# BosonHBC/BHRayTracer

Measured on AMD Instinct MI355X. Metric: Mrays/s (closest-hit + any-hit rays per second), with wall-clock per frame, higher is better.
Workload: dtype f32

## Files before the change

bhraytracer_amd/csrc/device_state.h:

```cpp
#pragma once
#include "dev_buf.h"

namespace bhrt {

struct DeviceQueues {
    hipStream_t stream = nullptr;
    hipEvent_t ev[2] = {nullptr, nullptr};
    hipStream_t stream2 = nullptr;
    std::vector<hipEvent_t> slow_events;
    hipStream_t stream3 = nullptr;
    hipEvent_t ev_shade = nullptr, ev_shadow[2] = {nullptr, nullptr};
    std::vector<hipEvent_t> ev_pool;
    DeviceQueues() = default;
    DeviceQueues(const DeviceQueues &) = delete;
    DeviceQueues &operator=(const DeviceQueues &) = delete;
    ~DeviceQueues()
    {
        if (ev_shade) (void)hipEventDestroy(ev_shade);
        for (int k = 0; k < 2; k++) if (ev_shadow[k]) (void)hipEventDestroy(ev_shadow[k]);
        if (stream3) (void)hipStreamDestroy(stream3);
        for (int k = 0; k < 2; k++) if (ev[k]) (void)hipEventDestroy(ev[k]);
        for (hipEvent_t e : ev_pool) (void)hipEventDestroy(e);
        for (hipEvent_t e : slow_events) (void)hipEventDestroy(e);
        if (stream2) (void)hipStreamDestroy(stream2);
// ... 22 lines not shown
            if (GatherSortPairs(nullptr, nullptr, nullptr, nullptr, cnt, nullptr, &sort_temp_bytes, 28, stream) != 0) { SetError("gather sort: temp size"); return BHRT_ERR_HIP; }
            BHRT_TRY(d_sort_temp.Reserve(std::max<size_t>(sort_temp_bytes, 16)));
            cap = cnt;
        }
        BHRT_TRY(d_cnt.Reserve(1));
        BHRT_TRY(d_cells.Reserve((size_t)BHRT_GATHER_CELLS + 1));
        BHRT_TRY(d_tile_sums.Reserve((size_t)(BHRT_GATHER_CELLS / kScanTile + kScanBlock)));
        return h_cnt ? BHRT_OK : h_cnt.Alloc(1);
    }
};

struct PhotonSlot {
    DevBuf<DPhoton> d_photons;
    uint32_t n_photons = 0;
    std::vector<HostPhoton> h_photons;
    DevBuf<float4> d_ph_hot, d_ph_cold, d_ph_dbox;
    PhotonMapDev pm = {};
    void Clear() { d_photons.Free(); d_ph_hot.Free(); d_ph_cold.Free(); d_ph_dbox.Free(); n_photons = 0; h_photons.clear(); pm = PhotonMapDev{}; }
};

struct DeviceState : DeviceQueues {
    int device = -1;
    uint32_t n_cus = 256;
    DevBuf<uint8_t> d_blob;
    DevBuf<int32_t> d_chain;
    DevBuf<float> d_aux;
    DevBuf<bhrt_texcolor> d_emission;
    bool emission_on = false;
    bool emission_textured = false;
    bool le_on = false;
    DevBuf<float> d_le;
    DevBuf<bhrt_material> d_mtl_ext;
    DevBuf<float> d_r0_ext;
    DevBuf<int32_t> d_fm_tab;
    FaceMtlTable fm = {nullptr, 0};
    DevScene S;
    ShutterInfo shutter = {};
    uint32_t cap_samples = 0, cap_rays = 0, cap_frames = 0;
    DevBuf<float> d_rayf[2];
    DevBuf<uint32_t> d_rayu[2];
    DevBuf<float> d_hitf;
    DevBuf<int32_t> d_hiti;
    DevBuf<float> d_shf;
    DevBuf<uint32_t> d_shu;
    DevBuf<uint32_t> d_fu;
    DevBuf<uint64_t> d_fcode;
    DevBuf<float> d_ff;
    DevBuf<float> d_samples;
    DevBuf<uint32_t> d_root;
    DevBuf<uint32_t> d_order;
    uint32_t order_shard_cap = 0;
    DevBuf<uint32_t> d_seg;
    DevBuf<uint32_t> d_park;
    DevBuf<float> d_slowf;
    DevBuf<uint32_t> d_slowu;
    DevBuf<float> d_shf2;
    DevBuf<uint32_t> d_shu2;
    DevBuf<uint32_t> d_order_sh;
    DevBuf<uint32_t> d_seg_sh;
    DevBuf<Counters> d_cnt_sh;
    DevBuf<Counters> d_cnt;
    PinnedBuf<HostCounters> h_pub;
    HostCounters *d_pub = nullptr;
    uint32_t pub_seq = 0;
    int timers = 0;
    struct PendingTimer { int e0, e1; double *acc; };
    std::vector<PendingTimer> ev_pending;
    std::vector<int> ev_free;
    PhotonSlot cmap, gmap;
    DevBuf<float> d_ph_frames;
    GatherWorkspace gw;
    struct Knobs {
        int stream_waves = -1;
        bool fused_camera = true;
        bool no_slow_queue = false;
        bool debug_slow = false, debug_gather = false, debug_drain = false;
        bool balance_host = false;
        int frame_cap = 0;
        int gather_lane_budget = 0;
        bool gather_counting_sort = false;
        bool shadow_overlap = true;
        bool fused_resolve = true;
        bool finish_misses = true;
        int gather_stats = 0;
        void FromEnv()
        {
            if (const char *e = getenv("BHRT_STREAM_WAVES")) stream_waves = atoi(e);
            if (const char *e = getenv("BHRT_FUSED_CAMERA")) fused_camera = atoi(e) != 0;
            no_slow_queue = getenv("BHRT_NO_SLOW_QUEUE") != nullptr;
            debug_slow = getenv("BHRT_DEBUG_SLOW") != nullptr; debug_gather = getenv("BHRT_DEBUG_GATHER") != nullptr; debug_drain = getenv("BHRT_DEBUG_DRAIN") != nullptr;
            if (const char *e = getenv("BHRT_PHOTON_BALANCE_HOST")) balance_host = atoi(e) != 0;
            if (const char *e = getenv("BHRT_GATHER_COUNTING_SORT")) gather_counting_sort = atoi(e) != 0;
            if (const char *e = getenv("BHRT_SHADOW_OVERLAP")) shadow_overlap = atoi(e) != 0;
            if (const char *e = getenv("BHRT_FUSED_RESOLVE")) fused_resolve = atoi(e) != 0;
            if (const char *e = getenv("BHRT_FINISH_MISSES")) finish_misses = atoi(e) != 0;
        }
    } knobs;
    uint64_t pass_hint_key = 0;
    uint32_t pass_hint = 0;
    uint64_t frames_seen_key = 0;
    double frames_seen = 0;
    size_t frame_px = 0;
    DevBuf<uint8_t> d_frame_rgb;
    DevBuf<float> d_frame_rad, d_frame_var;
    DevBuf<uint32_t> d_frame_cnt;
    DevBuf<uint8_t> d_ad;
    DevBuf<uint8_t> d_prog;
    uint64_t prog_session = 0;
    DevBuf<uint8_t> d_dn;
    DevBuf<float4> d_guides;
    struct MovingNodeSlot {
        PinnedBuf<uint32_t> h;
        DevBuf<uint32_t> d;
        hipEvent_t done = nullptr;
        bool used = false;
        MovingNodeSlot() = default;
        MovingNodeSlot(const MovingNodeSlot &) = delete;
        MovingNodeSlot &operator=(const MovingNodeSlot &) = delete;
        ~MovingNodeSlot() { if (done) (void)hipEventDestroy(done); }
    } moving_nodes[2];
    uint32_t moving_turn = 0;
    DevBuf<int32_t> d_moving_id;
    size_t api_cap = 0;
    DevBuf<float> d_api_f;
    DevBuf<int32_t> d_api_i;
};

void DestroyDeviceState(DeviceState *d)
{
    if (!d) return;
    if (d->device >= 0) (void)hipSetDevice(d->device);
    delete d;
}

}
```

bhraytracer_amd/csrc/kernels.hip:

```cpp
#include <hip/hip_runtime.h>

#include <stdlib.h>
#include <string.h>

#include <algorithm>
#include <type_traits>
#include <chrono>
#include <string>
#include <vector>

#include "bhrt.h"
#include "denoise.h"
#include "temporal.h"
#include "device_color24.h"
#include "device_photon.h"
#include "photon_host.h"
#include "scene_internal.h"

namespace bhrt {

#define HIP_CHECK(expr)                                                                                        \
    do {                                                                                                       \
        hipError_t e_ = (expr);                                                                                \
        if (e_ != hipSuccess) {                                                                                \
// ... 212 lines not shown
        else atomicOr(&cnt->overflow.v, 8u);
    }
}
__device__ inline uint32_t shading_class(uint32_t meta, const Hit &hit)
{
    const uint32_t kind = meta & 15u;
    const bool is_hit = hit.node >= 0;
    bool heavy = false;
    if (is_hit) {
        if (kind == RK_CAMERA) heavy = true;
        else if (kind == RK_GI) heavy = fabsf(hit.t) > BHRT_BIAS;
        else if (kind == RK_REFR_IN) heavy = hit.front != 0;
        else heavy = true;
    }
    return heavy ? RC_HEAVY : ((kind == RK_REFR_IN && is_hit) ? RC_MEDIUM : RC_LIGHT);
}
template <bool kTex>
__device__ inline void gi_miss(const DevScene &S, const float *gi_mult, float *gi, uint32_t owner, V3 d)
{
    const V3 mult = ld3i(gi_mult, owner);
    V3 outc = v3(0, 0, 0);
    if (d.x == d.y && d.x == 0) {
        outc = outc + v3(1.0f, 0.0f, 1.0f);
    } else {
        V3 env = (kTex ? sample_environment(S, S.environment, d) : ld3(S.environment.color)) * mult;
        if (!(isnan_f(env.x) || isnan_f(env.y) || isnan_f(env.z))) outc = outc + env;
    }
    if (isnan_f(outc.x)) outc = v3(1.0f, 0.0f, 1.0f);
    else outc = clamp_white(outc);
    st3(gi, owner, outc);
}

struct SlowQueue {
    RayQueue q;
    uint32_t cap;
};
constexpr uint32_t kSlowCap = 1u << 16;
template <bool kPark, bool kCamera, bool kMeshes = true>
__global__ void __launch_bounds__(kBlock) __attribute__((amdgpu_waves_per_eu(kPark ? 7 : 1, 8))) k_trace_closest(DevScene S, PassInfo P, RayQueue q, uint32_t n, int uniform_side, HitBuf h, RayOrder ord, Counters *cnt,
                                                          SlowQueue slow , const float *fin_gi_mult, float *fin_gi, uint32_t *fin_root)
{
    constexpr bool kFinish = kPark || !kMeshes;
    __shared__ bhrt_bvh_node nodelet[(kPark || !kMeshes) ? 1 : BHRT_LDS_NODES];
    const uint32_t i = blockIdx.x * blockDim.x + threadIdx.x;
    bool active = i < n;
    V3 o = v3(0, 0, 0), d = v3(0, 0, 1);
    uint32_t meta = 0;
    if (active) fetch_ray<kCamera>(S, P, q, i, o, d, meta);
    const bool has_meta = kCamera || q.meta;
    const int side = has_meta ? (int)((meta >> 4) & 3u) : uniform_side;
    const bool dead = has_meta && (meta & 15u) == RK_DEAD;
    Hit hit;
    uint32_t key = 0;
    bool is_slow = false;
    int parked = trace_closest<kMeshes>(S, o, d, side, hit, active && !dead, (kPark || !kMeshes) ? nullptr : nodelet, 0, kPark, kPark ? &key : nullptr,
                                        (uint16_t *)nullptr, 0, BHRT_LDS_NODES, kCamera, kPark ? &is_slow : nullptr);
    if (kPark && parked >= 0 && is_slow && slow.cap) {
        const uint32_t k = atomicAdd(&cnt->n_slow.v, 1u);
        if (k < slow.cap) {
            slow.q.ox[k] = o.x; slow.q.oy[k] = o.y; slow.q.oz[k] = o.z; slow.q.dx[k] = d.x; slow.q.dy[k] = d.y; slow.q.dz[k] = d.z;
            slow.q.frame[k] = kCamera ? i : q.frame[i];
            slow.q.meta[k] = meta;
            slow.q.rng_ctr[k] = (kCamera || (meta & 15u) == RK_GI) ? 0u : q.rng_ctr[i];
            active = false;
            parked = -1;
        }
    }
    if (kFinish && active && !dead && parked < 0 && hit.node < 0) {
        const uint32_t kind = meta & 15u;
        if (!kCamera && kind == RK_GI && fin_gi) {
            gi_miss<false>(S, fin_gi_mult, fin_gi, q.frame[i], d);
            active = false;
        } else if (kind == RK_CAMERA && fin_root) {
            uint32_t slot = i;
            if (!kCamera) slot = q.frame[i];
            fin_root[slot] = kNoRootFrame;
            active = false;
        }
    }
    if (active) { h.t[i] = hit.t; h.node[i] = hit.node; h.prim[i] = hit.prim; h.front[i] = hit.front | ((parked + 1) << 8); }
    if (kPark && parked >= 0) {
        ord.park_key[i] = key;
        if (!kCamera) ord.park_rank[i] = atomicAdd(&ord.park_bucket[key], 1u);
    }
    if (!ord.idx) return;
    uint32_t cls = RC_NONE;
    if (active && !dead) cls = parked >= 0 ? (uint32_t)RC_MESH : shading_class(meta, hit);
    file_ray(cls, i, (i >> 10) & (BHRT_ORDER_SHARDS - 1) , ord, cnt);
}
__device__ inline bool parked_entry(const RayOrder &ord, uint32_t b, uint32_t *s_seg, uint32_t &i, uint32_t first_entry = 0 )
{
    __syncthreads();
    if (threadIdx.x < 64) {
        const uint32_t l = threadIdx.x;
        const uint32_t a = l <= BHRT_ORDER_SHARDS ? ord.mesh_start[l] : 0xffffffffu;
        const uint32_t n_le = (uint32_t)__popcll(__ballot(l < BHRT_ORDER_SHARDS && a <= b));
        if (l == 0) *s_seg = n_le - 1;
    }
    __syncthreads();
    if (b >= ord.mesh_start[BHRT_ORDER_SHARDS]) return false;
    const uint32_t seg = *s_seg;
    const uint32_t local = (b - ord.mesh_start[seg]) * kBlock + first_entry + threadIdx.x;
    const bool active = local < ord.mesh_count[seg];
    i = active ? ord.idx[((size_t)RC_MESH * BHRT_ORDER_SHARDS + seg) * ord.shard_cap + local] : 0xffffffffu;
    return true;
}
#ifndef BHRT_XCD_LOCAL
#define BHRT_XCD_LOCAL 0
#endif
__device__ inline bool xcd_slice(uint32_t b, uint32_t nb, uint32_t &slice)
{
    slice = b;
#if BHRT_XCD_LOCAL
    constexpr uint32_t G = BHRT_XCD_LOCAL, span = 8 * G;
    const uint32_t chunk = b / span, in = b % span;
    if ((chunk + 1) * span <= nb) slice = chunk * span + (in & 7u) * G + (in >> 3);
#endif
    return b < nb;
}
__global__ void __launch_bounds__(kBlock) k_park_scatter(RayOrder ord)
{
    __shared__ uint32_t s_seg;
    uint32_t i;
    for (uint32_t b = blockIdx.x; parked_entry(ord, b, &s_seg, i); b += gridDim.x)
        if (i != 0xffffffffu) ord.park_sorted[ord.park_bucket[ord.park_key[i]] + ord.park_rank[i]] = i;
}
constexpr uint32_t kMeshNodelet = 256;
#ifndef BHRT_MESH_BLOCK
#define BHRT_MESH_BLOCK 64
#endif
constexpr int kMeshBlock = BHRT_MESH_BLOCK;
template <bool kCamera, int kPath, bool kLS = false>
__global__ void __launch_bounds__(kCamera ? kBlock : kMeshBlock, kPath == 1 ? 6 : 4 ) k_trace_mesh(DevScene S, PassInfo P, RayQueue q, HitBuf h, RayOrder ord, Counters *cnt)
{
    typedef typename std::conditional<kPath == 2, uint32_t, uint16_t>::type PathT;
    constexpr int kTB = kCamera ? kBlock : kMeshBlock;
    __shared__ bhrt_bvh_node nodelet[kPath ? 1 : kMeshNodelet];
    __shared__ PathT path[kPath ? 33 * kTB : 1];
    __shared__ uint32_t s_seg;
    bool active;
    uint32_t i;
    uint32_t slice;
    if (kCamera) {
        if (!xcd_slice(blockIdx.x, ord.mesh_start[BHRT_ORDER_SHARDS], slice)) return;
        if (!parked_entry(ord, slice, &s_seg, i)) return;
        active = i != 0xffffffffu;
        if (!active) i = 0;
    } else {
        const uint32_t total = ord.mesh_count[BHRT_ORDER_SHARDS];
        if (!xcd_slice(blockIdx.x, (total + kTB - 1) / kTB, slice)) return;
        const uint32_t k = slice * kTB + threadIdx.x;
        active = k < total;
        i = active ? ord.park_sorted[k] : 0u;
    }
    V3 o = v3(0, 0, 0), d = v3(0, 0, 1);
    uint32_t meta = 0;
    Hit hit = {BHRT_BIGFLOAT, -1, -1, 1};
    int start = 0;
    if (active) {
        fetch_ray<kCamera>(S, P, q, i, o, d, meta);
        hit.t = h.t[i]; hit.node = h.node[i]; hit.prim = h.prim[i];
        const int fw = h.front[i];
        hit.front = fw & 0xff;
        start = (fw >> 8) - 1;
    }
    trace_closest<true, PathT, kLS>(S, o, d, (int)((meta >> 4) & 3u), hit, active, kPath ? nullptr : nodelet, active ? start : S.n_nodes, false, nullptr,
// ... 59 lines not shown
            }
            if (!pending) { h.t[i] = hit.t; h.node[i] = hit.node; h.prim[i] = hit.prim; h.front[i] = hit.front; have = false; }
        }
        if (!exhausted) {
            const uint64_t idle = __ballot(!have);
            const uint32_t n_idle = (uint32_t)__popcll(idle);
            if (n_idle >= (uint32_t)kStreamRefill) {
                uint32_t base = 0;
                if (lane == 0) base = atomicAdd(&cnt->mesh_cursor.v, n_idle);
                base = (uint32_t)__builtin_amdgcn_readfirstlane((int)base);
                exhausted = base + n_idle >= total;
#ifdef BHRT_DEBUG_STREAM
                dbg[5]++;
#endif
#ifdef BHRT_DEBUG_DRAIN
                if (exhausted && !told && lane == 0) { atomicMin(&g_stream_t[1], wall_clock64()); }
                told = told || exhausted;
#endif
                const uint32_t k = base + (uint32_t)__popcll(idle & ((1ull << lane) - 1ull));
                if (!have && k < total) {
                    i = ord.park_sorted[k];
                    hit.t = h.t[i]; hit.node = h.node[i]; hit.prim = h.prim[i];
                    const int fw = h.front[i];
                    hit.front = fw & 0xff;
                    n = (fw >> 8) - 1;
                    side = (int)(((q.meta ? q.meta[i] : 0u) >> 4) & 3u);
                    have = true;
                    pending = true;
                }
            }
        }
        if (!__ballot(have)) break;
        const uint64_t waiting = __ballot(pending);
        if (!__ballot(W.st != 3) && waiting) {
            const int nn = __builtin_amdgcn_readlane(n, __ffsll((unsigned long long)waiting) - 1);
            if (nn != cur_n) { cur_n = nn; M = mesh_ref(S, S.nodes[cur_n].mesh); }
        }
        if (pending && n == cur_n) {
            V3 lp = v3(q.ox[i], q.oy[i], q.oz[i]), ld = v3(q.dx[i], q.dy[i], q.dz[i]);
            local_ray(S, n, lp, ld);
            walk_begin(M, W, lp, ld, hit.t);
            pending = false;
        }
        const int n_wait = __popcll(__ballot(pending));
#ifdef BHRT_DEBUG_STREAM
        c_mark = __builtin_readcyclecounter();
#endif
        for (;;) {
            const int nD = __popcll(__ballot(W.st == 0)), nL = __popcll(__ballot(W.st == 1)), nC = __popcll(__ballot(W.st == 2));
            const int walking = nD + nL + nC;
            if (walking == 0 || (!exhausted && 64 - walking - n_wait >= kStreamRefill)) break;
#ifdef BHRT_DEBUG_STREAM
#if BHRT_FUSED_CLIMB
            dbg[0]++; dbg[1] += walking; dbg[2] += (nD >= nL && nD > 0) ? nD : nL;
            if (nD >= nL && nD > 0) dbg[6]++; else if (nL > 0) dbg[7]++;
#else
            dbg[0]++; dbg[1] += walking; dbg[2] += (nD >= nL && nD >= nC) ? nD : (nL >= nC ? nL : nC);
            if (nD >= nL && nD >= nC) dbg[6]++; else if (nL >= nC) dbg[7]++;
#endif
#endif
#ifdef BHRT_DEBUG_STREAM
            const unsigned long long r0 = __builtin_readcyclecounter();
#endif
            walk_round<PathT, kLS>(M, W, side, hit.t, hit.prim, hit.front, stack, 64u, nD, nL, nC);
#ifdef BHRT_DEBUG_STREAM
            if (nD >= nL && nD > 0) dbg[4] += __builtin_readcyclecounter() - r0;
#endif
        }
#ifdef BHRT_DEBUG_STREAM
        { const unsigned long long c = __builtin_readcyclecounter(); dbg[3] += c - c_mark; c_mark = c; }
#endif
    }
#ifdef BHRT_DEBUG_STREAM
    if (lane == 0) for (int k = 0; k < 8; k++) atomicAdd(&g_stream_dbg[k], dbg[k]);
#endif
#ifdef BHRT_DEBUG_DRAIN
    if (lane == 0) atomicMax(&g_stream_t[2], wall_clock64());
#endif
}
__global__ void __launch_bounds__(kBlock) k_file_parked(RayQueue q, HitBuf h, RayOrder ord, Counters *cnt)
{
    __shared__ uint32_t s_seg;
    uint32_t i;
    if (!parked_entry(ord, blockIdx.x, &s_seg, i)) return;
    const bool active = i != 0xffffffffu;
    uint32_t cls = RC_NONE;
    if (active) {
        Hit hit;
        hit.t = h.t[i]; hit.node = h.node[i]; hit.prim = h.prim[i]; hit.front = h.front[i];
        cls = shading_class(q.meta[i], hit);
    }
    file_ray(cls, active ? i : 0u, blockIdx.x & (BHRT_ORDER_SHARDS - 1), ord, cnt);
}

__global__ void __launch_bounds__(64) k_trace_slow(DevScene S, SlowQueue slow, uint32_t a, uint32_t b, HitBuf h)
{
    __shared__ CoopLds lds;
    __builtin_amdgcn_s_setprio(3);
    const uint32_t i = a + blockIdx.x;
    if (i >= b) return;
    const V3 o = v3(slow.q.ox[i], slow.q.oy[i], slow.q.oz[i]), d = v3(slow.q.dx[i], slow.q.dy[i], slow.q.dz[i]);
    const uint32_t meta = slow.q.meta[i];
    Hit hit;
#ifdef BHRT_DEBUG_LONG_RAYS
    const unsigned long long c0 = wall_clock64();
#endif
    trace_closest_coop(S, lds, o, d, (int)((meta >> 4) & 3u), hit);
#ifdef BHRT_DEBUG_LONG_RAYS
    const double ms = (double)(wall_clock64() - c0) / 1e5;
    if (threadIdx.x == 0 && ms > 5.0) printf("slow ray %u: %.1f ms o=(%.9g %.9g %.9g) d=(%.9g %.9g %.9g) side %u -> node %d prim %d t %.9g\n", i, ms, o.x, o.y, o.z, d.x, d.y, d.z, (meta >> 4) & 3u, hit.node, hit.prim, hit.t);
#endif
    if (threadIdx.x == 0) { h.t[i] = hit.t; h.node[i] = hit.node; h.prim[i] = hit.prim; h.front[i] = hit.front; }
}
__global__ void __launch_bounds__(kBlock) k_inject_slow(RayQueue sq, HitBuf sh, uint32_t src0, uint32_t m, RayQueue q, HitBuf h, uint32_t dst0)
{
    const uint32_t k = blockIdx.x * blockDim.x + threadIdx.x;
    if (k >= m) return;
    const uint32_t a = src0 + k, b = dst0 + k;
    q.ox[b] = sq.ox[a]; q.oy[b] = sq.oy[a]; q.oz[b] = sq.oz[a]; q.dx[b] = sq.dx[a]; q.dy[b] = sq.dy[a]; q.dz[b] = sq.dz[a];
    q.frame[b] = sq.frame[a]; q.meta[b] = sq.meta[a]; q.rng_ctr[b] = sq.rng_ctr[a];
    h.t[b] = sh.t[a]; h.node[b] = sh.node[a]; h.prim[b] = sh.prim[a]; h.front[b] = sh.front[a];
}
static inline uint32_t kFileAllBlocks(uint32_t first, uint32_t n) { return (n - (first & ~63u) + kBlock - 1) / kBlock; }
__global__ void __launch_bounds__(kBlock) k_file_all(RayQueue q, HitBuf h, uint32_t first, uint32_t n, RayOrder ord, Counters *cnt)
{
    const uint32_t i = (first & ~63u) + blockIdx.x * blockDim.x + threadIdx.x;
    uint32_t cls = RC_NONE;
    if (i >= first && i < n) {
        Hit hit;
        hit.t = h.t[i]; hit.node = h.node[i]; hit.prim = h.prim[i]; hit.front = h.front[i];
        cls = shading_class(q.meta[i], hit);
    }
    file_ray(cls, i, (i >> 10) & (BHRT_ORDER_SHARDS - 1), ord, cnt);
}

template <bool kMeshes>
__global__ void __launch_bounds__(kBlock) k_trace_shadow(DevScene S, ShadowQueue q, uint32_t n, const uint32_t *n_dev, float *vis)
{
    const uint32_t i = blockIdx.x * blockDim.x + threadIdx.x;
    if (n_dev) n = min(n, *n_dev);
    if (i >= n) return;
    const V3 o = v3(q.ox[i], q.oy[i], q.oz[i]), d = v3(q.dx[i], q.dy[i], q.dz[i]);
    const float v = kMeshes ? trace_shadow_t<0>(S, o, d, q.tmax[i]) : trace_shadow_t<3>(S, o, d, q.tmax[i]);
    vis[q.frame ? q.frame[i] : i] = v;
}
__global__ void __launch_bounds__(kBlock) k_trace_shadow_park(DevScene S, ShadowQueue q, uint32_t n, const uint32_t *n_dev, float *vis, RayOrder ord, Counters *cnt)
{
    const uint32_t i = blockIdx.x * blockDim.x + threadIdx.x;
    if (n_dev) n = min(n, *n_dev);
    if (blockIdx.x * blockDim.x >= n) return;
    float v = 1.f;
    if (i < n) {
        v = trace_shadow_t<1>(S, v3(q.ox[i], q.oy[i], q.oz[i]), v3(q.dx[i], q.dy[i], q.dz[i]), q.tmax[i]);
        if (v != 2.f) vis[q.frame[i]] = v;
    }
    file_ray(v == 2.f ? (uint32_t)RC_MESH : (uint32_t)RC_NONE, i, (i >> 10) & (BHRT_ORDER_SHARDS - 1), ord, cnt);
}
#ifndef BHRT_SHADOW_BLOCK
#define BHRT_SHADOW_BLOCK 64
#endif
constexpr int kShadowBlock = BHRT_SHADOW_BLOCK;
template <int kPath, bool kLS = false>
__global__ void __launch_bounds__(kShadowBlock) k_shadow_mesh(DevScene S, ShadowQueue q, float *vis, RayOrder ord)
{
    typedef typename std::conditional<kPath == 2, uint32_t, uint16_t>::type PathT;
    __shared__ uint32_t s_seg;
    __shared__ PathT path[kPath ? 33 * kShadowBlock : 1];
    constexpr uint32_t kParts = kBlock / kShadowBlock;
    uint32_t i, slice;
    if (!xcd_slice(blockIdx.x / kParts, ord.mesh_start[BHRT_ORDER_SHARDS], slice)) return;
    if (!parked_entry(ord, slice, &s_seg, i, (blockIdx.x % kParts) * kShadowBlock)) return;
    if (i == 0xffffffffu) return;
    vis[q.frame[i]] = trace_shadow_t<2, PathT, kLS>(S, v3(q.ox[i], q.oy[i], q.oz[i]), v3(q.dx[i], q.dy[i], q.dz[i]), q.tmax[i], kPath ? path + threadIdx.x : (PathT *)nullptr, kShadowBlock);
}

// ... 2022 lines not shown
            cur ^= 1;
            pass_steps++;
        }
        if (sh_overlap) for (int k = 0; k < 2; k++) if (sh_pending[k]) HIP_CHECK(hipStreamWaitEvent(D->stream, D->ev_shadow[k], 0));
        return BHRT_OK;
    }

    int Begin()
    {
        HIP_CHECK(hipMemsetAsync(D->d_cnt, 0, sizeof(Counters), D->stream));
        if (lens) {
            Timer t(D, &st->seconds_other);
            if (shutter) hipLaunchKernelGGL(k_shutter_rays, dim3((n_cur + kBlock - 1) / kBlock), dim3(kBlock), 0, D->stream, D->S, P, D->shutter, V.Q[0], n_cur);
            else hipLaunchKernelGGL(k_lens_rays, dim3((n_cur + kBlock - 1) / kBlock), dim3(kBlock), 0, D->stream, D->S, P, V.Q[0], n_cur);
            t.Stop();
        }
        if (D->stream2) HIP_CHECK(hipStreamSynchronize(D->stream2));
        if (D->stream3) HIP_CHECK(hipStreamSynchronize(D->stream3));
        return BHRT_OK;
    }

    int MoveInSetAside()
    {
        injected = false;
        n_extra = 0;
        if (n_cur == 0) {
            const auto w0 = std::chrono::steady_clock::now();
            HIP_CHECK(hipStreamSynchronize(D->stream2));
            if (D->knobs.debug_slow)
                fprintf(stderr, "slow rays: %u moved in after wave step %u, waited %.1f ms for their hits, pass time so far %.1f ms\n", slow_pending, pass_steps, MsSince(w0), MsSince(wall0));
            n_cur = slow_pending - slow_injected;
            hipLaunchKernelGGL(k_inject_slow, dim3((n_cur + kBlock - 1) / kBlock), dim3(kBlock), 0, D->stream, V.slowq.q, V.slow_hits, slow_injected, n_cur, V.Q[cur], V.HB, 0u);
            pass_deferred += n_cur;
            slow_injected = slow_pending;
            slow_batch_next = slow_batches.size();
            injected = true;
        } else if (!first_step && n_cur >= kInjectMinRays) {
            uint32_t upto = slow_injected;
            size_t b = slow_batch_next;
            while (b < slow_batches.size() && slow_batches[b].step + 2 <= pass_steps) { upto = slow_batches[b].end; b++; }
            if (upto > slow_injected && (uint64_t)n_cur + (upto - slow_injected) <= D->cap_rays) {
                HIP_CHECK(hipStreamWaitEvent(D->stream, slow_batches[b - 1].done, 0));
                n_extra = upto - slow_injected;
                hipLaunchKernelGGL(k_inject_slow, dim3((n_extra + kBlock - 1) / kBlock), dim3(kBlock), 0, D->stream, V.slowq.q, V.slow_hits, slow_injected, n_extra, V.Q[cur], V.HB, n_cur);
                if (D->knobs.debug_slow) fprintf(stderr, "slow rays: %u ride along with wave step %u (%u rays)\n", n_extra, pass_steps, n_cur);
                pass_deferred += n_extra;
                slow_injected = upto;
                slow_batch_next = b;
            }
        }
        return BHRT_OK;
    }

    int TraceClosest()
    {
        const RayOrder &RO = V.RO;
        const bool fused = Fused();
        if (fused) {
        } else if (injected) {
            Timer t(D, &st->seconds_trace_closest);
            hipLaunchKernelGGL(k_file_all, dim3((n_cur + kBlock - 1) / kBlock), dim3(kBlock), 0, D->stream, V.Q[cur], V.HB, 0u, n_cur, RO, D->d_cnt);
            t.Stop();
        } else {
            Timer t(D, &st->seconds_trace_closest);
            const SlowQueue no_slow = {V.slowq.q, 0u};
            if (meshes) BHRT_TRY(TraceThroughMeshes());
            else hipLaunchKernelGGL(ClosestKernel(false, CamStep(), false), dim3((n_cur + kBlock - 1) / kBlock), dim3(kBlock), 0, D->stream, D->S, P, V.Q[cur], n_cur, 0, V.HB, RO, D->d_cnt, no_slow, finish ? V.F.gi_mult : nullptr, finish ? V.F.gi : nullptr, finish ? root_of : nullptr);
            t.Stop();
        }
        if (n_extra) hipLaunchKernelGGL(k_file_all, dim3(kFileAllBlocks(n_cur, n_cur + n_extra)), dim3(kBlock), 0, D->stream, V.Q[cur], V.HB, n_cur, n_cur + n_extra, RO, D->d_cnt);
        if (!fused) {
            st->launches_trace_closest++;
            hipLaunchKernelGGL(k_order_prefix, dim3(1), dim3(128), 0, D->stream, D->d_cnt, RO);
        }
        return BHRT_OK;
    }

    int TraceThroughMeshes()
    {
        const RayOrder &RO = V.RO;
        const bool cam_step = CamStep();
        const dim3 tg((n_cur + kBlock - 1) / kBlock), tb(kBlock);
        const uint32_t n_buckets = 1u << BHRT_PARK_KEY_BITS;
        if (!cam_step) HIP_CHECK(hipMemsetAsync(RO.park_bucket, 0, n_buckets * sizeof(uint32_t), D->stream));
        hipLaunchKernelGGL(ClosestKernel(true, cam_step, true), tg, tb, 0, D->stream, D->S, P, V.Q[cur], n_cur, 0, V.HB, RO, D->d_cnt, V.slowq, finish ? V.F.gi_mult : nullptr, finish ? V.F.gi : nullptr, finish ? root_of : nullptr);
        hipLaunchKernelGGL(k_mesh_prefix, dim3(1), dim3(64), 0, D->stream, D->d_cnt, RO);
        if (!cam_step) {
            const dim3 pg(std::min<uint32_t>(tg.x + BHRT_ORDER_SHARDS, 4096u));
            LaunchExclusiveScan(D->stream, RO.park_bucket, n_buckets, RO.park_bucket + n_buckets);
            hipLaunchKernelGGL(k_park_scatter, pg, tb, 0, D->stream, RO);
        }
        if (sh_wait_n) {
            HIP_CHECK(hipEventRecord(D->ev_shade, D->stream));
            BHRT_TRY(LaunchQueuedAnyHit(D->ev_shade));
        }
        if (!cam_step && path_mode != 0 && stream_waves > 0) {
            BHRT_TRY(DebugDrainReset());
            hipLaunchKernelGGL(StreamKernel(path_mode, ls), dim3(std::min<uint32_t>((n_cur + 63) / 64, stream_waves)), dim3(64), 0, D->stream, D->S, V.Q[cur], V.HB, RO, D->d_cnt);
            BHRT_TRY(DebugDrainReport(D, n_cur));
        } else
            hipLaunchKernelGGL(MeshKernel(cam_step, path_mode, ls), cam_step ? dim3(tg.x + BHRT_ORDER_SHARDS)  : dim3((n_cur + kMeshBlock - 1) / kMeshBlock),
                               cam_step ? tb : dim3(kMeshBlock), 0, D->stream, D->S, P, V.Q[cur], V.HB, RO, D->d_cnt);
        if (!cam_step) hipLaunchKernelGGL(k_file_parked, dim3(tg.x + BHRT_ORDER_SHARDS), tb, 0, D->stream, V.Q[cur], V.HB, RO, D->d_cnt);
        return BHRT_OK;
    }

    int Shade()
    {
        const bool fused = Fused();
        seq = ++D->pub_seq;
        Timer t(D, &st->seconds_shade, 0);
        const dim3 sg((n_cur + n_extra + kShadeBlock - 1) / kShadeBlock + (fused ? 0 : 3 * BHRT_ORDER_SHARDS)), sb(kShadeBlock);
        const int par = (int)(pass_steps & 1u);
        if (sh_wait_n) { HIP_CHECK(hipEventRecord(D->ev_shade, D->stream)); BHRT_TRY(LaunchQueuedAnyHit(D->ev_shade)); }
        if (sh_overlap && sh_pending[par]) { HIP_CHECK(hipStreamWaitEvent(D->stream, D->ev_shadow[par], 0)); sh_pending[par] = false; }
        hipLaunchKernelGGL(ShadeKernel(fused, CamStep(), tex, V.F.le != nullptr, V.F.fm.tab != nullptr, gg), sg, sb, 0, D->stream, D->S, R, P, V.Q[cur], V.HB, n_cur + n_extra, V.Q[cur ^ 1], (sh_overlap && par) ? V.SQ2 : V.SQ, V.F, D->d_samples, root_of, D->d_cnt, V.RO, D->d_pub, seq);
        t.Stop();
        if (sh_overlap) HIP_CHECK(hipEventRecord(D->ev_shade, D->stream));
        return BHRT_OK;
    }

    void LaunchAnyHit(hipStream_t stream, const ShadowQueue &sq, uint32_t n, const uint32_t *n_dev, const RayOrder &order, Counters *counters)
    {
        Timer t(D, &st->seconds_trace_shadow, 1, stream);
        const dim3 hg((n + kBlock - 1) / kBlock), hb(kBlock);
        if (meshes) {
            hipLaunchKernelGGL(k_trace_shadow_park, hg, hb, 0, stream, D->S, sq, n, n_dev, V.F.vis, order, counters);
            hipLaunchKernelGGL(k_mesh_prefix, dim3(1), dim3(64), 0, stream, counters, order);
            hipLaunchKernelGGL(AnyHitMeshKernel(path_mode, ls), dim3((hg.x + BHRT_ORDER_SHARDS) * (kBlock / kShadowBlock)), dim3(kShadowBlock), 0, stream, D->S, sq, V.F.vis, order);
        } else hipLaunchKernelGGL(k_trace_shadow<false>, hg, hb, 0, stream, D->S, sq, n, n_dev, V.F.vis);
        t.Stop();
    }

    int LaunchQueuedAnyHit(hipEvent_t after)
    {
        if (!sh_wait_n) return BHRT_OK;
        const int par = sh_wait_par; const uint32_t n_sh = sh_wait_n;
        sh_wait_n = 0;
        HIP_CHECK(hipStreamWaitEvent(D->stream3, after, 0));
        LaunchAnyHit(D->stream3, par ? V.SQ2 : V.SQ, n_sh, nullptr, V.RO_sh, D->d_cnt_sh);
        HIP_CHECK(hipEventRecord(D->ev_shadow[par], D->stream3));
        sh_pending[par] = true;
        return BHRT_OK;
    }

    int ReadCounters()
    {
        BHRT_TRY(WaitPublished(D, seq));
        hc = *D->h_pub;
        FlushTimers(D);
        if (hc.overflow) { overflow = true; return BHRT_OK; }
        if (first_step) {
            const uint64_t valid_px = P.list ? P.n_pixels : CountValidPixels(P, P.n_pixels);
            pass_closest = valid_px * (uint64_t)P.spp;
            pass_camera = pass_closest;
            first_step = false;
        } else if (!injected) pass_closest += n_cur;
        if (hc.n_shadow) { pass_shadow += hc.n_shadow; st->launches_trace_shadow++; }
        frame_marks.push_back(hc.n_frames);
        return BHRT_OK;
    }

    int TraceSetAside()
    {
        slow_pending = std::min<uint32_t>(hc.n_slow, kSlowCap);
        if (slow_pending <= slow_traced) return BHRT_OK;
        const uint32_t cnt_new = slow_pending - slow_traced;
        hipLaunchKernelGGL(k_trace_slow, dim3(cnt_new), dim3(64), 0, D->stream2, D->S, V.slowq, slow_traced, slow_pending, V.slow_hits);
        if (D->knobs.debug_slow) fprintf(stderr, "slow rays: %u set aside in wave step %u at %.1f ms\n", cnt_new, pass_steps, MsSince(wall0));
        slow_traced = slow_pending;
        const size_t bi = slow_batches.size();
        if (bi >= D->slow_events.size()) { hipEvent_t e = nullptr; HIP_CHECK(hipEventCreateWithFlags(&e, hipEventDisableTiming)); D->slow_events.push_back(e); }
        HIP_CHECK(hipEventRecord(D->slow_events[bi], D->stream2));
        slow_batches.push_back({slow_pending, pass_steps, D->slow_events[bi]});
        return BHRT_OK;
    }

    int QueueAnyHit()
    {
        if (!hc.n_shadow) return BHRT_OK;
        sh_wait_par = (int)(pass_steps & 1u); sh_wait_n = hc.n_shadow;
        if (hc.n_next == 0) BHRT_TRY(LaunchQueuedAnyHit(D->ev_shade));
        return BHRT_OK;
    }
};

// ... 282 lines not shown
    const int rc = render(&local);
    if (stats) *stats = local;
    return rc;
}

struct FrameStage {
    uint8_t *rgb8; float *radiance, *variance; uint32_t *count;
    uint8_t *d_rgb8 = nullptr; float *d_radiance = nullptr, *d_variance = nullptr; uint32_t *d_count = nullptr;
    size_t npix = 0;
    int Reserve(bhrt_scene *scene)
    {
        DeviceState *D = scene->dev;
        npix = (size_t)scene->flat.hdr()->camera.width * scene->flat.hdr()->camera.height;
        if (D->frame_px < npix) {
            D->frame_px = 0;
            BHRT_TRY(D->d_frame_rgb.Reserve(npix * 3));
            BHRT_TRY(D->d_frame_rad.Reserve(npix * 3));
            D->frame_px = npix;
        }
        if (variance) BHRT_TRY(D->d_frame_var.Reserve(npix * 3));
        if (count) BHRT_TRY(D->d_frame_cnt.Reserve(npix));
        d_rgb8 = rgb8 ? D->d_frame_rgb.p : nullptr; d_radiance = radiance ? D->d_frame_rad.p : nullptr;
        d_variance = variance ? D->d_frame_var.p : nullptr; d_count = count ? D->d_frame_cnt.p : nullptr;
        return BHRT_OK;
    }
    int Upload(hipStream_t s) const
    {
        if (rgb8) HIP_CHECK(hipMemcpyAsync(d_rgb8, rgb8, npix * 3, hipMemcpyHostToDevice, s));
        if (radiance) HIP_CHECK(hipMemcpyAsync(d_radiance, radiance, npix * 12, hipMemcpyHostToDevice, s));
        if (variance) HIP_CHECK(hipMemcpyAsync(d_variance, variance, npix * 12, hipMemcpyHostToDevice, s));
        if (count) HIP_CHECK(hipMemcpyAsync(d_count, count, npix * 4, hipMemcpyHostToDevice, s));
        return BHRT_OK;
    }
    int Download(hipStream_t s) const
    {
        if (rgb8) HIP_CHECK(hipMemcpyAsync(rgb8, d_rgb8, npix * 3, hipMemcpyDeviceToHost, s));
        if (radiance) HIP_CHECK(hipMemcpyAsync(radiance, d_radiance, npix * 12, hipMemcpyDeviceToHost, s));
        if (variance) HIP_CHECK(hipMemcpyAsync(variance, d_variance, npix * 12, hipMemcpyDeviceToHost, s));
        if (count) HIP_CHECK(hipMemcpyAsync(count, d_count, npix * 4, hipMemcpyDeviceToHost, s));
        HIP_CHECK(hipStreamSynchronize(s));
        return BHRT_OK;
    }
};

void *SceneStream(const bhrt_scene *scene) { return scene && scene->dev ? (void *)scene->dev->stream : nullptr; }
int SceneDevice(const bhrt_scene *scene) { return scene && scene->dev ? scene->dev->device : -1; }
int RenderArgsCheck(bhrt_scene *scene, const bhrt_opts *opts)
{
    BHRT_CHECK_LENS(scene, opts);
    BHRT_CHECK_GLOBAL(scene);
    if (opts->photon_map && !(scene->dev && scene->dev->cmap.d_photons)) { SetError("photon_map = 1 needs bhrt_photon_build first"); return BHRT_ERR_ARG; }
    PassInfo P;
    uint64_t owned_pixels = 0;
    return FramePassInfo(scene, *opts, P, owned_pixels);
}

}

using namespace bhrt;

extern "C" {

int bhrt_device_count(int *n)
try {
    if (!n) { SetError("null argument"); return BHRT_ERR_ARG; }
    int c = 0;
    hipError_t e = hipGetDeviceCount(&c);
    if (e != hipSuccess) { *n = 0; SetError(std::string("hipGetDeviceCount: ") + hipGetErrorString(e)); return BHRT_ERR_NO_DEVICE; }
    *n = c;
    return BHRT_OK;
} catch (...) { return bhrt::AbiException(); }

int bhrt_scene_knob(bhrt_scene *scene, const char *name, int value)
try {
    int rc = EnsureUploaded(scene);
    if (rc) return rc;
    if (!name || value < 0) { SetError("knob: bad arguments"); return BHRT_ERR_ARG; }
    if (!strcmp(name, "frame_cap")) scene->dev->knobs.frame_cap = value;
    else if (!strcmp(name, "gather_lane_budget")) scene->dev->knobs.gather_lane_budget = value;
    else if (!strcmp(name, "gather_stats")) scene->dev->knobs.gather_stats = value;
    else if (!strcmp(name, "shadow_overlap")) scene->dev->knobs.shadow_overlap = value != 0;
    else if (!strcmp(name, "fused_resolve")) scene->dev->knobs.fused_resolve = value != 0;
    else if (!strcmp(name, "finish_misses")) scene->dev->knobs.finish_misses = value != 0;
    else { SetError(std::string("knob: unknown name ") + name); return BHRT_ERR_ARG; }
    return BHRT_OK;
} catch (...) { return bhrt::AbiException(); }

int bhrt_scene_upload(bhrt_scene *scene, int device)
try {
    if (!scene) { SetError("null scene"); return BHRT_ERR_ARG; }
    if (scene->dev && scene->dev->device == device) { HIP_CHECK(hipSetDevice(device)); return BHRT_OK; }
    if (scene->dev && scene->prog.open && scene->dev->prog_session == scene->prog.id) {
        SetError("bhrt_scene_upload: a progressive session of this scene holds its state on device " + std::to_string(scene->dev->device) + ": bhrt_progressive_end first");
        return BHRT_ERR_ARG;
    }
    if (scene->dev && TemporalSessionHoldsBuffers(scene->temporal)) {
        SetError("bhrt_scene_upload: a temporal session of this scene holds its images on device " + std::to_string(scene->dev->device) + ": bhrt_temporal_end first");
        return BHRT_ERR_ARG;
    }
    int count = 0;
    if (hipGetDeviceCount(&count) != hipSuccess || count <= 0) { SetError("no HIP device available (this path has no CPU fallback)"); return BHRT_ERR_NO_DEVICE; }
    if (device < 0 || device >= count) { SetError("device index out of range"); return BHRT_ERR_ARG; }
    if (scene->max_bvh_depth > 64) { SetError("BVH deeper than 64 levels: the stackless trail holds 64"); return BHRT_ERR_UNSUPPORTED; }
    if (scene->dev) { DestroyDeviceState(scene->dev); scene->dev = nullptr; }
    HIP_CHECK(hipSetDevice(device));
    DeviceState *D = new DeviceState;
    D->knobs.FromEnv();
    D->device = device;
    scene->dev = D;
    {
        int cus = 0;
        if (hipDeviceGetAttribute(&cus, hipDeviceAttributeMultiprocessorCount, device) == hipSuccess && cus > 0) D->n_cus = (uint32_t)cus;
    }
    const std::vector<uint8_t> &blob = scene->flat.blob;
    const bhrt_flat_header *H = scene->flat.hdr();
    HIP_CHECK(hipStreamCreate(&D->stream));
    HIP_CHECK(hipEventCreate(&D->ev[0]));
    HIP_CHECK(hipEventCreate(&D->ev[1]));
    BHRT_TRY(D->d_blob.Reserve(blob.size()));
    HIP_CHECK(hipMemcpy(D->d_blob, blob.data(), blob.size(), hipMemcpyHostToDevice));
    std::vector<int32_t> chain((size_t)std::max<uint32_t>(H->n_nodes, 1) * BHRT_MAX_NODE_DEPTH, 0);
    const bhrt_node *nodes = (const bhrt_node *)(blob.data() + H->off_nodes);
    for (uint32_t n = 0; n < H->n_nodes; n++) {
        int k = nodes[n].depth - 1, c = (int)n;
        while (c >= 0 && k >= 0) { chain[(size_t)n * BHRT_MAX_NODE_DEPTH + k] = c; c = nodes[c].parent; k--; }
    }
    BHRT_TRY(D->d_chain.Reserve(chain.size()));
    HIP_CHECK(hipMemcpy(D->d_chain, chain.data(), chain.size() * sizeof(int32_t), hipMemcpyHostToDevice));
    BHRT_TRY(D->d_cnt.Reserve(1));
    if (H->n_meshes > 0) {
        BHRT_TRY(D->d_slowf.Reserve((size_t)kSlowCap * 7));
        BHRT_TRY(D->d_slowu.Reserve((size_t)kSlowCap * 6));
        {
            int lo_prio = 0, hi_prio = 0;
            (void)hipDeviceGetStreamPriorityRange(&lo_prio, &hi_prio);
            HIP_CHECK(hipStreamCreateWithPriority(&D->stream2, hipStreamNonBlocking, hi_prio));
            {
                HIP_CHECK(hipStreamCreateWithPriority(&D->stream3, hipStreamNonBlocking, hi_prio));
                HIP_CHECK(hipEventCreateWithFlags(&D->ev_shade, hipEventDisableTiming));
                for (int k = 0; k < 2; k++) HIP_CHECK(hipEventCreateWithFlags(&D->ev_shadow[k], hipEventDisableTiming));
                BHRT_TRY(D->d_seg_sh.Reserve(2 * BHRT_ORDER_SHARDS + 2));
                BHRT_TRY(D->d_cnt_sh.Reserve(1));
                HIP_CHECK(hipMemset(D->d_cnt_sh, 0, sizeof(Counters)));
            }
        }
    }
    BHRT_TRY(D->d_seg.Reserve(11 * BHRT_ORDER_SHARDS + 3));
    BHRT_TRY(D->h_pub.Alloc(1, hipHostMallocMapped));
    memset(D->h_pub, 0, sizeof(HostCounters));
    HIP_CHECK(hipHostGetDevicePointer((void **)&D->d_pub, D->h_pub, 0));
    DevScene &S = D->S;
    S.blob = D->d_blob;
    S.nodes = (const bhrt_node *)(D->d_blob + H->off_nodes);
    S.meshes = (const bhrt_mesh *)(D->d_blob + H->off_meshes);
    S.materials = (const bhrt_material *)(D->d_blob + H->off_materials);
    S.lights = (const bhrt_light *)(D->d_blob + H->off_lights);
    S.texmaps = (const bhrt_texmap *)(D->d_blob + H->off_texmaps);
    S.textures = (const bhrt_texture *)(D->d_blob + H->off_textures);
    S.chain = D->d_chain;
    S.n_nodes = (int32_t)H->n_nodes; S.n_lights = (int32_t)H->n_lights;
    S.all_light_intensity = H->all_light_intensity;
    {
        const bhrt_material *mats = (const bhrt_material *)(scene->flat.blob.data() + H->off_materials);
        const size_t n_cam = (size_t)std::max<uint32_t>(H->n_nodes, 1) * BHRT_MAX_NODE_DEPTH * 3;
        std::vector<float> aux(H->n_materials + H->n_lights + 1 + n_cam, 0.f);
        FillCamChain(scene->flat, aux.data() + H->n_materials + H->n_lights + 1);
// ... 1649 lines not shown
```

Measured before the change: 7119.

## Add optional camera-step streaming path and grid-stride parked-ray filing

Makes k_file_parked a grid-stride loop over parked slices, capping its grid at a configurable block count (default 4096) instead of launching one block per slice. It also adds an opt-in camera_stream mode, off by default. In that mode the camera closest-hit kernel writes parked rays into the queue, a new k_park_compact kernel builds the sorted park list, and the persistent stream kernel then traverses them instead of the mesh kernel. The cap is meant to cut block-launch overhead on large secondary passes, at the cost of less parallelism when there are many slices.

```diff
diff --git a/bhraytracer_amd/csrc/device_state.h b/bhraytracer_amd/csrc/device_state.h
--- a/bhraytracer_amd/csrc/device_state.h
+++ b/bhraytracer_amd/csrc/device_state.h
@@ -128,6 +128,8 @@
         bool shadow_overlap = true;
         bool fused_resolve = true;
         bool finish_misses = true;
+        int file_parked_blocks = 4096;
+        bool camera_stream = false;
         int gather_stats = 0;
         void FromEnv()
         {
@@ -140,6 +142,8 @@
             if (const char *e = getenv("BHRT_SHADOW_OVERLAP")) shadow_overlap = atoi(e) != 0;
             if (const char *e = getenv("BHRT_FUSED_RESOLVE")) fused_resolve = atoi(e) != 0;
             if (const char *e = getenv("BHRT_FINISH_MISSES")) finish_misses = atoi(e) != 0;
+            if (const char *e = getenv("BHRT_FILE_PARKED_BLOCKS")) file_parked_blocks = atoi(e) > 0 ? atoi(e) : 0;
+            if (const char *e = getenv("BHRT_CAMERA_STREAM")) camera_stream = atoi(e) != 0;
         }
     } knobs;
     uint64_t pass_hint_key = 0;
diff --git a/bhraytracer_amd/csrc/kernels.hip b/bhraytracer_amd/csrc/kernels.hip
--- a/bhraytracer_amd/csrc/kernels.hip
+++ b/bhraytracer_amd/csrc/kernels.hip
@@ -318,6 +318,7 @@
     if (kPark && parked >= 0) {
         ord.park_key[i] = key;
         if (!kCamera) ord.park_rank[i] = atomicAdd(&ord.park_bucket[key], 1u);
+        if (kCamera && q.ox) { q.ox[i] = o.x; q.oy[i] = o.y; q.oz[i] = o.z; q.dx[i] = d.x; q.dy[i] = d.y; q.dz[i] = d.z; q.meta[i] = meta; }
     }
     if (!ord.idx) return;
     uint32_t cls = RC_NONE;
@@ -543,15 +544,28 @@
 {
     __shared__ uint32_t s_seg;
     uint32_t i;
-    if (!parked_entry(ord, blockIdx.x, &s_seg, i)) return;
-    const bool active = i != 0xffffffffu;
-    uint32_t cls = RC_NONE;
-    if (active) {
-        Hit hit;
-        hit.t = h.t[i]; hit.node = h.node[i]; hit.prim = h.prim[i]; hit.front = h.front[i];
-        cls = shading_class(q.meta[i], hit);
-    }
-    file_ray(cls, active ? i : 0u, blockIdx.x & (BHRT_ORDER_SHARDS - 1), ord, cnt);
+    for (uint32_t b = blockIdx.x; parked_entry(ord, b, &s_seg, i); b += gridDim.x) {
+        const bool active = i != 0xffffffffu;
+        uint32_t cls = RC_NONE;
+        if (active) {
+            Hit hit;
+            hit.t = h.t[i]; hit.node = h.node[i]; hit.prim = h.prim[i]; hit.front = h.front[i];
+            cls = shading_class(q.meta[i], hit);
+        }
+        file_ray(cls, active ? i : 0u, b & (BHRT_ORDER_SHARDS - 1) , ord, cnt);
+    }
+}
+__global__ void __launch_bounds__(kBlock) k_park_compact(RayOrder ord)
+{
+    __shared__ uint32_t s_seg;
+    uint32_t i;
+    for (uint32_t b = blockIdx.x; parked_entry(ord, b, &s_seg, i); b += gridDim.x) {
+        if (i == 0xffffffffu) continue;
+        const uint32_t seg = (uint32_t)__builtin_amdgcn_readfirstlane((int)s_seg);
+        uint32_t first = 0;
+        for (uint32_t s = 0; s < seg; s++) first += ord.mesh_count[s];
+        ord.park_sorted[first + (b - ord.mesh_start[seg]) * kBlock + threadIdx.x] = i;
+    }
 }
 
 __global__ void __launch_bounds__(64) k_trace_slow(DevScene S, SlowQueue slow, uint32_t a, uint32_t b, HitBuf h)
@@ -2740,26 +2754,32 @@
         const bool cam_step = CamStep();
         const dim3 tg((n_cur + kBlock - 1) / kBlock), tb(kBlock);
         const uint32_t n_buckets = 1u << BHRT_PARK_KEY_BITS;
+        const bool cam_stream = cam_step && path_mode != 0 && stream_waves > 0 && D->knobs.camera_stream;
+        const bool queued = !cam_step || cam_stream;
+        const dim3 pg(std::min<uint32_t>(tg.x + BHRT_ORDER_SHARDS, 4096u));
         if (!cam_step) HIP_CHECK(hipMemsetAsync(RO.park_bucket, 0, n_buckets * sizeof(uint32_t), D->stream));
-        hipLaunchKernelGGL(ClosestKernel(true, cam_step, true), tg, tb, 0, D->stream, D->S, P, V.Q[cur], n_cur, 0, V.HB, RO, D->d_cnt, V.slowq, finish ? V.F.gi_mult : nullptr, finish ? V.F.gi : nullptr, finish ? root_of : nullptr);
+        hipLaunchKernelGGL(ClosestKernel(true, cam_step, true), tg, tb, 0, D->stream, D->S, P, queued ? V.Q[cur] : RayQueue{}, n_cur, 0, V.HB, RO, D->d_cnt, V.slowq, finish ? V.F.gi_mult : nullptr, finish ? V.F.gi : nullptr, finish ? root_of : nullptr);
         hipLaunchKernelGGL(k_mesh_prefix, dim3(1), dim3(64), 0, D->stream, D->d_cnt, RO);
         if (!cam_step) {
-            const dim3 pg(std::min<uint32_t>(tg.x + BHRT_ORDER_SHARDS, 4096u));
             LaunchExclusiveScan(D->stream, RO.park_bucket, n_buckets, RO.park_bucket + n_buckets);
             hipLaunchKernelGGL(k_park_scatter, pg, tb, 0, D->stream, RO);
-        }
+        } else if (cam_stream)
+            hipLaunchKernelGGL(k_park_compact, pg, tb, 0, D->stream, RO);
         if (sh_wait_n) {
             HIP_CHECK(hipEventRecord(D->ev_shade, D->stream));
             BHRT_TRY(LaunchQueuedAnyHit(D->ev_shade));
         }
-        if (!cam_step && path_mode != 0 && stream_waves > 0) {
+        if (queued && path_mode != 0 && stream_waves > 0) {
             BHRT_TRY(DebugDrainReset());
             hipLaunchKernelGGL(StreamKernel(path_mode, ls), dim3(std::min<uint32_t>((n_cur + 63) / 64, stream_waves)), dim3(64), 0, D->stream, D->S, V.Q[cur], V.HB, RO, D->d_cnt);
             BHRT_TRY(DebugDrainReport(D, n_cur));
         } else
             hipLaunchKernelGGL(MeshKernel(cam_step, path_mode, ls), cam_step ? dim3(tg.x + BHRT_ORDER_SHARDS)  : dim3((n_cur + kMeshBlock - 1) / kMeshBlock),
                                cam_step ? tb : dim3(kMeshBlock), 0, D->stream, D->S, P, V.Q[cur], V.HB, RO, D->d_cnt);
-        if (!cam_step) hipLaunchKernelGGL(k_file_parked, dim3(tg.x + BHRT_ORDER_SHARDS), tb, 0, D->stream, V.Q[cur], V.HB, RO, D->d_cnt);
+        if (queued) {
+            const uint32_t slices = tg.x + BHRT_ORDER_SHARDS, cap = (uint32_t)D->knobs.file_parked_blocks;
+            hipLaunchKernelGGL(k_file_parked, dim3(cap ? std::min(slices, cap) : slices), tb, 0, D->stream, V.Q[cur], V.HB, RO, D->d_cnt);
+        }
         return BHRT_OK;
     }
 
@@ -3208,6 +3228,8 @@
     else if (!strcmp(name, "shadow_overlap")) scene->dev->knobs.shadow_overlap = value != 0;
     else if (!strcmp(name, "fused_resolve")) scene->dev->knobs.fused_resolve = value != 0;
     else if (!strcmp(name, "finish_misses")) scene->dev->knobs.finish_misses = value != 0;
+    else if (!strcmp(name, "file_parked_blocks")) scene->dev->knobs.file_parked_blocks = value;
+    else if (!strcmp(name, "camera_stream")) scene->dev->knobs.camera_stream = value != 0;
     else { SetError(std::string("knob: unknown name ") + name); return BHRT_ERR_ARG; }
     return BHRT_OK;
 } catch (...) { return bhrt::AbiException(); }
```

After: 7139 (median of 4 runs). Within noise of the previous version (+0.3%).
